# Madhudorai/encodec-pytorch

Hardware: AMD Instinct MI355X
Metric: audio-seconds/sec EnCodec24k train step, batch 32x1s (higher is better)
Workload: dtype f32; 1 GPU; config 3: 24 kHz mono full GAN (MS-STFT disc + Balancer); global_batch=32, parallelism=dp1

## Files before the change

### encodec-pytorch_amd/csrc/conv2d.h

```cpp
#pragma once
#include "common.h"

constexpr int NT = 256;
constexpr int DPER = 8;

struct C2Geo {
    int B, Ci, T2, Fi, Co, Fo, KT, KF, sf, dt, pt, pf;
};
static inline bool geo_ok(const C2Geo& g) {
    return g.B > 0 && g.Ci > 0 && g.T2 > 0 && g.Fi > 0 && g.Co > 0 && g.Fo > 0 && g.KT > 0 && g.KF > 0 &&
           g.sf > 0 && g.dt > 0 && g.pt >= 0 && g.pf >= 0 &&
           g.Fo == (g.Fi + 2 * g.pf - g.KF) / g.sf + 1 && g.T2 + 2 * g.pt - g.dt * (g.KT - 1) == g.T2;
}

static inline int c2_rows(int BN, int len) { return (len + BN - 2) / len + 1; }

static inline int c2_ck(int VC, int per_ch, int budget = 12288) {
    int ck = budget / per_ch;
    if (ck > 32) ck = 32;
    int vce = (VC + 1) & ~1;
    if (ck > vce) ck = vce;
    ck &= ~1;
    if (ck < 2) ck = 2;
    for (int c = ck; c >= 2; c -= 2)
        if (VC % c == 0 && c * 2 >= ck) return c;
    return ck;
}

static inline int quad_ck(int VC, int NR, int RL, int MQ, int CKM) {
    const int quads = NR * (((RL + 3) & ~3) >> 2);
    int ck = MQ * NT / quads;
    ck = std::min(ck, CKM);
    ck = std::min(ck, (VC + 1) & ~1);
    ck &= ~1;
    return ck;
}

extern int g_c2_select;
bool rw_pays(int64_t items, int64_t positions, double ratio);

ENCX_DEV f32x4 quad_abs(f32x4 v, int o, int last) {
    const int sh = o < 0 ? o : (o > last ? o - last : 0);
    const int n = sh < 0 ? -sh : sh;
    const bool b1 = n & 1, b2 = n & 2;
    f32x4 r;
    if (sh >= 0) {
        const float t0 = b1 ? v[1] : v[0], t1 = b1 ? v[2] : v[1], t2 = b1 ? v[3] : v[2], t3 = b1 ? 0.f : v[3];
        r[0] = b2 ? t2 : t0;
        r[1] = b2 ? t3 : t1;
        r[2] = b2 ? 0.f : t2;
        r[3] = b2 ? 0.f : t3;
    } else {
        const float t0 = b1 ? 0.f : v[0], t1 = b1 ? v[0] : v[1], t2 = b1 ? v[1] : v[2], t3 = b1 ? v[2] : v[3];
        r[0] = b2 ? 0.f : t0;
        r[1] = b2 ? 0.f : t1;
        r[2] = b2 ? t0 : t2;
        r[3] = b2 ? t1 : t3;
    }
    return r;
}

ENCX_DEV int rw_first_slot(int wave) { return wave * (int)gridDim.x + xcd_linear_id(); }
```

### encodec-pytorch_amd/csrc/conv2d_fwd.hip

```cpp
#include "common.h"
#include "conv2d.h"
#include "prof.h"

namespace {

struct C2Fwd {
    C2Geo g;
    const float* x;
    const float* wf;
    const float* bias;
    float* y;
    int act;
    int CK, NR, RL;
};

template <int BM, int BN, int WM, int WN, int KFC = 0>
__global__ __launch_bounds__(NT) void c2_fwd_kernel(C2Fwd a) {
    constexpr int TM = BM / WM / 32, TN = BN / WN / 32;
    extern __shared__ float smem[];
    const C2Geo g = a.g;
    const int CK = a.CK, NR = a.NR, RL = a.RL, KF = g.KF, S = g.sf;
    const int VC = g.Ci * g.KT, XR = NR * RL;
    float* Xs = smem;
    float* Ws = smem + CK * XR;
    const int tid = threadIdx.x, lane = tid & 63, wave = tid >> 6;
    const int wm0 = (wave / WN) * TM * 32, wn0 = (wave % WN) * TN * 32;
    const int h = lane >> 5, l32 = lane & 31;
    const int b = blockIdx.z, n0 = blockIdx.x * BN, co0 = blockIdx.y * BM;
    const int Nall = g.T2 * g.Fo, nend = min(Nall, n0 + BN);
    const int tf = n0 / g.Fo, f0 = n0 - tf * g.Fo;
    const int nr = (nend - 1) / g.Fo - tf + 1;
    int boff[TN];
#pragma unroll
    for (int j = 0; j < TN; ++j) {
        const int n = n0 + wn0 + j * 32 + l32;
        boff[j] = 0;
        if (n < nend) {
            const int tr = n / g.Fo, f = n - tr * g.Fo, rs = tr - tf;
            boff[j] = rs * RL + (f - (rs ? 0 : f0)) * S;
        }
    }
    f32x16 acc[TM][TN];
#pragma unroll
    for (int i = 0; i < TM; ++i)
#pragma unroll
        for (int j = 0; j < TN; ++j) acc[i][j] = (f32x16){0};
    const float* xb = a.x + (int64_t)b * g.Ci * g.T2 * g.Fi;
    int2* rtab = (int2*)(Ws + KF * CK * BM);
    for (int gr = tid; gr < VC * NR; gr += NT) {
        const int vc = gr / NR, rs = gr - vc * NR, ci = vc / g.KT, kt = vc - ci * g.KT;
        const int row = tf + rs + kt * g.dt - g.pt, pos0 = (rs ? 0 : f0) * S - g.pf;
        const bool ok = rs < nr && row >= 0 && row < g.T2;
        rtab[gr] = make_int2(ok ? (ci * g.T2 + row) * g.Fi + pos0 : 0, ok ? pos0 : -(1 << 30));
    }
    const int dr = NT / RL, dw = NT - dr * RL, r_init = tid / RL, w_init = tid - r_init * RL;
    const int wcol = tid & (BM - 1);
    for (int c0 = 0; c0 < VC; c0 += CK) {
        __syncthreads();
        {
            const int nrows = min(CK, VC - c0) * NR, items = CK * XR;
            int r = r_init, w = w_init;
            for (int i0 = 0; i0 < items; i0 += NT * DPER) {
                int rq[DPER], wq[DPER];
#pragma unroll
                for (int q = 0; q < DPER; ++q) {
                    rq[q] = r;
                    wq[q] = w;
                    w += dw;
                    r += dr;
                    if (w >= RL) {
                        w -= RL;
                        ++r;
                    }
                }
                int2 e[DPER];
#pragma unroll
                for (int q = 0; q < DPER; ++q) e[q] = rtab[c0 * NR + (rq[q] < nrows ? rq[q] : 0)];
                float v[DPER];
#pragma unroll
                for (int q = 0; q < DPER; ++q) {
                    const int pos = e[q].y + wq[q];
                    const bool ok = rq[q] < nrows && pos >= 0 && pos < g.Fi;
                    const float t = xb[ok ? e[q].x + wq[q] : 0];
                    v[q] = ok ? t : 0.f;
                }
#pragma unroll
                for (int q = 0; q < DPER; ++q) {
                    const int i = i0 + q * NT + tid;
                    if (i < items) Xs[i] = v[q];
                }
            }
        }
        {
            const int items = KF * CK * BM, rows = (VC - c0) * KF, co = co0 + wcol;
            const float* wsrc = a.wf + (int64_t)c0 * KF * g.Co + co;
            for (int i0 = 0; i0 < items; i0 += NT * DPER) {
                float v[DPER];
#pragma unroll
                for (int q = 0; q < DPER; ++q) {
                    const int rr = (i0 + q * NT + tid) / BM;
                    const bool ok = rr < rows && co < g.Co;
                    const float t = wsrc[ok ? (int64_t)rr * g.Co : 0];
                    v[q] = ok ? t : 0.f;
                }
#pragma unroll
                for (int q = 0; q < DPER; ++q) {
                    const int i = i0 + q * NT + tid;
                    if (i < items) Ws[i] = v[q];
                }
            }
        }
        __syncthreads();
        if constexpr (KFC > 0) {
            for (int cp = 0; cp < CK; cp += 2) {
                const float* wk = Ws + (cp + h) * KFC * BM + wm0 + l32;
                const float* xk = Xs + (cp + h) * XR;
#pragma unroll
                for (int kf = 0; kf < KFC; ++kf) {
                    float av[TM], bv[TN];
#pragma unroll
                    for (int i = 0; i < TM; ++i) av[i] = wk[kf * BM + i * 32];
#pragma unroll
                    for (int j = 0; j < TN; ++j) bv[j] = xk[boff[j] + kf];
#pragma unroll
                    for (int i = 0; i < TM; ++i)
#pragma unroll
                        for (int j = 0; j < TN; ++j) acc[i][j] = mfma32(av[i], bv[j], acc[i][j]);
                }
            }
        } else {
            for (int kf = 0; kf < KF; ++kf) {
                const float* wk = Ws + (h * KF + kf) * BM + wm0 + l32;
                const float* xk = Xs + h * XR + kf;
                for (int cp = 0; cp < CK; cp += 2) {
                    float av[TM], bv[TN];
#pragma unroll
                    for (int i = 0; i < TM; ++i) av[i] = wk[cp * KF * BM + i * 32];
#pragma unroll
                    for (int j = 0; j < TN; ++j) bv[j] = xk[cp * XR + boff[j]];
#pragma unroll
                    for (int i = 0; i < TM; ++i)
#pragma unroll
                        for (int j = 0; j < TN; ++j) acc[i][j] = mfma32(av[i], bv[j], acc[i][j]);
                }
            }
        }
    }
#pragma unroll
    for (int i = 0; i < TM; ++i)
#pragma unroll
        for (int j = 0; j < TN; ++j) {
            const int n = n0 + wn0 + j * 32 + l32;
#pragma unroll
            for (int r = 0; r < 16; ++r) {
                const int co = co0 + wm0 + i * 32 + mfma_row(r, lane);
                const float bco = a.bias ? a.bias[co < g.Co ? co : g.Co - 1] : 0.f;
                if (co < g.Co && n < nend) {
                    float v = acc[i][j][r] + bco;
                    if (a.act) v = lrelu(v);
                    a.y[((int64_t)b * g.Co + co) * Nall + n] = v;
                }
            }
        }
}

template <int BN, int KFC, int MQ, int CKM, int OCC = 1>
__global__ __launch_bounds__(NT, OCC) void c2_fwdr_kernel(C2Fwd a) {
    constexpr int BM = 32, TN = BN / 128, MW = (KFC * CKM * BM / 4 + NT - 1) / NT;
    extern __shared__ float smem[];
    const C2Geo g = a.g;
    const int CK = a.CK, NR = a.NR, RL = a.RL, S = g.sf;
    const int RLp = (RL + 3) & ~3, NQ = RLp >> 2;
    const int VC = g.Ci * g.KT, XR = NR * RLp, WQ = KFC * CK * BM / 4;
    float* Xs = smem;
    float* Ws = smem + CK * XR;
    int2* rtab = (int2*)(Ws + KFC * CK * BM);
    const int tid = threadIdx.x, lane = tid & 63, wave = tid >> 6;
    const int h = lane >> 5, l32 = lane & 31;
    const TileId tile = xcd_tile();
    const int b = tile.z, n0 = tile.x * BN, co0 = tile.y * BM;
    const int wn0 = wave * TN * 32;
    const int Nall = g.T2 * g.Fo, nend = min(Nall, n0 + BN);
    const int tf = n0 / g.Fo, f0 = n0 - tf * g.Fo;
    const int nr = (nend - 1) / g.Fo - tf + 1;
    const int base0 = ((f0 * S - g.pf) & ~3), baseN = ((-g.pf) & ~3);
    int boff[TN];
#pragma unroll
    for (int j = 0; j < TN; ++j) {
        const int n = n0 + wn0 + j * 32 + l32;
        boff[j] = 0;
        if (n < nend) {
            const int tr = n / g.Fo, f = n - tr * g.Fo, rs = tr - tf;
            boff[j] = rs * RLp + f * S - g.pf - (rs ? baseN : base0);
        }
    }
    f32x16 acc[TN];
#pragma unroll
    for (int j = 0; j < TN; ++j) acc[j] = (f32x16){0};
    const int64_t xtot = (int64_t)g.B * g.Ci * g.T2 * g.Fi;
    const float* xb = a.x + (int64_t)b * g.Ci * g.T2 * g.Fi;
    const int64_t xleft = xtot - (int64_t)b * g.Ci * g.T2 * g.Fi;
    for (int gr = tid; gr < VC * NR; gr += NT) {
        const int vc = gr / NR, rs = gr - vc * NR, ci = vc / g.KT, kt = vc - ci * g.KT;
        const int row = tf + rs + kt * g.dt - g.pt, base = rs ? baseN : base0;
        const bool ok = rs < nr && row >= 0 && row < g.T2;
        rtab[gr] = make_int2(ok ? (ci * g.T2 + row) * g.Fi + base : 0, ok ? base : -(1 << 30));
    }
    __syncthreads();
    const int rows = CK * NR;
    const int dr = NT / NQ, dq = NT - dr * NQ, r_init = tid / NQ, q_init = tid - r_init * NQ;
    f32x4 xv[MQ], wv[MW];
    int xmask[MQ], xdst[MQ];
    auto fetch = [&](int c0) {
        const int nrows = min(CK, VC - c0) * NR;
        int r = r_init, q = q_init;
#pragma unroll
        for (int u = 0; u < MQ; ++u) {
            const bool live = r < nrows;
            const int2 e = rtab[c0 * NR + (live ? r : 0)];
            const int col = e.y + 4 * q;
            const bool any = live && col >= 0 && col < g.Fi;
            int off = any ? e.x + 4 * q : 0;
            if (off > xleft - 4) off = (int)xleft - 4;
            xv[u] = ld4u(xb + off);
            const int sh = (any ? e.x + 4 * q : 0) - off;
            xmask[u] = any ? (min(g.Fi - col, 4) | (sh << 4)) : 0;
            xdst[u] = r < rows ? r * RLp + 4 * q : -1;
            q += dq;
            r += dr;
            if (q >= NQ) {
                q -= NQ;
                ++r;
            }
        }
        const float* wsrc = a.wf + (int64_t)c0 * KFC * g.Co + co0;
        const int wrows = (VC - c0) * KFC;
#pragma unroll
        for (int u = 0; u < MW; ++u) {
            const int j = u * NT + tid, rr = j >> 3, col = (j & 7) * 4;
            const bool ok = j < WQ && rr < wrows && co0 + col + 3 < g.Co;
            wv[u] = ld4u(wsrc + (ok ? (int64_t)rr * g.Co + col : 0));
            if (!ok) wv[u] = (f32x4){0.f, 0.f, 0.f, 0.f};
        }
    };
    fetch(0);
    for (int c0 = 0; c0 < VC; c0 += CK) {
        __syncthreads();
#pragma unroll
        for (int u = 0; u < MQ; ++u) {
            const int m = xmask[u], nv = m & 15, sh = m >> 4;
            f32x4 v = xv[u];
            if (sh) {
                const f32x4 t = v;
#pragma unroll
                for (int k = 0; k < 4; ++k) v[k] = k + sh < 4 ? (k + sh == 1 ? t[1] : k + sh == 2 ? t[2] : t[3]) : 0.f;
            }
#pragma unroll
            for (int k = 0; k < 4; ++k) v[k] = k < nv ? v[k] : 0.f;
            if (xdst[u] >= 0) *(f32x4*)(Xs + xdst[u]) = v;
        }
#pragma unroll
        for (int u = 0; u < MW; ++u) {
            const int j = u * NT + tid, rr = j >> 3, col = (j & 7) * 4;
            if (j < WQ && rr < (VC - c0) * KFC && co0 + col + 3 >= g.Co)
                for (int k = 0; k < 4; ++k)
                    wv[u][k] = co0 + col + k < g.Co ? a.wf[((int64_t)c0 * KFC + rr) * g.Co + co0 + col + k] : 0.f;
            if (j < WQ) *(f32x4*)(Ws + rr * BM + col) = wv[u];
        }
        __syncthreads();
        if (c0 + CK < VC) fetch(c0 + CK);
#pragma unroll 2
        for (int cp = 0; cp < CK; cp += 2) {
            const float* wk = Ws + (cp + h) * KFC * BM + l32;
            const float* xk = Xs + (cp + h) * XR;
#pragma unroll
            for (int kf = 0; kf < KFC; ++kf) {
                const float av = wk[kf * BM];
                float bv[TN];
#pragma unroll
                for (int j = 0; j < TN; ++j) bv[j] = xk[boff[j] + kf];
#pragma unroll
                for (int j = 0; j < TN; ++j) acc[j] = mfma32(av, bv[j], acc[j]);
            }
        }
    }
#pragma unroll
    for (int j = 0; j < TN; ++j) {
        const int n = n0 + wn0 + j * 32 + l32;
#pragma unroll
        for (int r = 0; r < 16; ++r) {
            const int co = co0 + mfma_row(r, lane);
            const float bco = a.bias ? a.bias[co < g.Co ? co : g.Co - 1] : 0.f;
            if (co < g.Co && n < nend) {
                float v = acc[j][r] + bco;
                if (a.act) v = lrelu(v);
                a.y[((int64_t)b * g.Co + co) * Nall + n] = v;
            }
        }
    }
}

struct C2FwdR {
    C2Geo g;
    const float* x;
    const float* wf;
    const float* bias;
    float* y;
    int act;
    int F4;
    int tiles;
};
template <int KF, int S, int WQ, int NWV>
__global__ __launch_bounds__(NWV * 64) void c2_fwd_rw_kernel(C2FwdR a) {
    constexpr int NE = 4 * WQ, KT = 3;
    extern __shared__ float smem[];
    const C2Geo g = a.g;
    float* Ws = smem;
    float* Bs = smem + g.Ci * KT * KF * 32;
    for (int i = threadIdx.x; i < g.Ci * KT * KF * 32; i += NWV * 64) {
        const int co = i & 31, r = i >> 5;
        Ws[i] = co < g.Co ? a.wf[r * g.Co + co] : 0.f;
    }
    if (threadIdx.x < 32) Bs[threadIdx.x] = (a.bias && (int)threadIdx.x < g.Co) ? a.bias[threadIdx.x] : 0.f;
    __syncthreads();
    const int lane = threadIdx.x & 63, wave = threadIdx.x >> 6, h = lane >> 5, l = lane & 31;
    const int quads = g.B * g.T2 * a.F4;
    const int plane = g.T2 * g.Fi, xlast = g.B * g.Ci * plane - 4;
    const int CP = g.Ci >> 1;
    const int cstride = 2 * plane;
    struct Geo {
        int t, b, f0;
        int rb[KT];
        uint32_t msk[KT];
        bool fix;
    };
    auto geo = [&](int tile) {
        Geo q;
        const int qd = min(tile * 32 + l, quads - 1);
        const int fq = qd % a.F4, bt = qd / a.F4;
        q.t = bt % g.T2;
        q.b = bt / g.T2;
        q.f0 = 4 * fq;
        const int col0 = S * q.f0 - g.pf;
        uint32_t cmask = 0;
#pragma unroll
        for (int e = 0; e < NE; ++e) cmask |= (col0 + e >= 0 && col0 + e < g.Fi) ? (1u << e) : 0u;
        bool clean = true;
#pragma unroll
        for (int kt = 0; kt < KT; ++kt) {
            const int row = q.t + kt * g.dt - g.pt;
            const bool ok = row >= 0 && row < g.T2;
            q.rb[kt] = (q.b * g.Ci + h) * plane + (ok ? row : 0) * g.Fi + col0;
            q.msk[kt] = ok ? cmask : 0u;
            clean = clean && q.msk[kt] == (1u << NE) - 1;
        }
        q.fix = !__all(clean);
        return q;
    };
    auto load = [&](f32x4* w, const Geo& q, int c, int kt) {
        const int base = q.rb[kt] + c * cstride;
#pragma unroll
        for (int w4 = 0; w4 < WQ; ++w4) w[w4] = ld4u(a.x + min(max(base + 4 * w4, 0), xlast));
    };
    f32x4 wb[KT][WQ];
    auto wcol = [&](int c, int kt) { return Ws + ((2 * c + h) * KT + kt) * KF * 32 + l; };
    const int stride = gridDim.x * NWV;
    int tile = rw_first_slot(wave);
    if (tile < a.tiles) load(wb[0], geo(tile), 0, 0);
    for (; tile < a.tiles; tile += stride) {
        const Geo cur = geo(tile);
        const int t = cur.t, b = cur.b, f0 = cur.f0;
        f32x16 acc[4];
#pragma unroll
        for (int j = 0; j < 4; ++j) acc[j] = (f32x16){0};
        for (int c = 0; c < CP; ++c) {
#pragma unroll
            for (int kt = 0; kt < KT; ++kt) {
                const int nk = kt + 1 < KT ? kt + 1 : 0;
                if (kt + 1 < KT) load(wb[nk], cur, c, nk);
                else if (c + 1 < CP) load(wb[0], cur, c + 1, 0);
                else load(wb[0], geo(tile + stride < a.tiles ? tile + stride : tile), 0, 0);
                f32x4* w = wb[kt];
                if (cur.fix) {
                    const int base = cur.rb[kt] + c * cstride;
#pragma unroll
                    for (int q = 0; q < WQ; ++q) {
                        const int o = base + 4 * q;
                        if (__any(o < 0 || o > xlast)) w[q] = quad_abs(w[q], o, xlast);
#pragma unroll
                        for (int e = 0; e < 4; ++e)
                            if (!((cur.msk[kt] >> (4 * q + e)) & 1u)) w[q][e] = 0.f;
                    }
                }
                const float* wk = wcol(c, kt);
#pragma unroll
                for (int kf = 0; kf < KF; ++kf) {
                    const float av = wk[kf * 32];
#pragma unroll
                    for (int j = 0; j < 4; ++j) {
                        const int r = S * j + kf;
                        acc[j] = mfma32(av, w[r >> 2][r & 3], acc[j]);
                    }
                }
            }
        }
        if (tile * 32 + l < quads) {
#pragma unroll
            for (int r = 0; r < 16; ++r) {
                const int co = mfma_row(r, lane);
                if (co >= g.Co) continue;
                const float bco = Bs[co];
                f32x4 v;
#pragma unroll
                for (int j = 0; j < 4; ++j) {
                    const float u = acc[j][r] + bco;
                    v[j] = a.act ? lrelu(u) : u;
                }
                float* dst = a.y + (((int64_t)b * g.Co + co) * g.T2 + t) * g.Fo + f0;
                if (f0 + 4 <= g.Fo) {
                    *(f32x4u*)dst = v;
                } else {
#pragma unroll
                    for (int j = 0; j < 4; ++j)
                        if (f0 + j < g.Fo) dst[j] = v[j];
                }
            }
        }
    }
}


template <int KT, int KF, int S>
__global__ __launch_bounds__(256) void c2_co1_fwd(C2Fwd a) {
    const C2Geo g = a.g;
    __shared__ float part[4][64];
    const int lane = threadIdx.x & 63, cg = threadIdx.x >> 6;
    const int plane = g.T2 * g.Fo, p = blockIdx.x * 64 + lane, b = blockIdx.y;
    const int pc = p < plane ? p : plane - 1;
    const int t = pc / g.Fo, fo = pc - t * g.Fo;
    const int64_t xplane = (int64_t)g.T2 * g.Fi;
    const int cper = (g.Ci + 3) >> 2, c0 = cg * cper, c1 = min(g.Ci, c0 + cper);
    const int fb = fo * S - g.pf;
    float acc = 0.f;
    for (int ci = c0; ci < c1; ++ci) {
        const float* xc = a.x + ((int64_t)b * g.Ci + ci) * xplane;
        const float* w = a.wf + ci * KT * KF;
#pragma unroll
        for (int kt = 0; kt < KT; ++kt) {
            const int tr = t + kt * g.dt - g.pt;
            const bool rok = tr >= 0 && tr < g.T2;
            const float* row = xc + (int64_t)(rok ? tr : 0) * g.Fi;
#pragma unroll
            for (int kf = 0; kf < KF; ++kf) {
                const int f = fb + kf;
                const bool ok = rok && f >= 0 && f < g.Fi;
                const float v = row[ok ? f : 0];
                acc = fmaf(w[kt * KF + kf], ok ? v : 0.f, acc);
            }
        }
    }
    part[cg][lane] = acc;
    __syncthreads();
    if (cg == 0 && p < plane) {
        float v = ((part[0][lane] + part[1][lane]) + part[2][lane]) + part[3][lane];
        if (a.bias) v += a.bias[0];
        a.y[(int64_t)b * plane + p] = a.act ? lrelu(v) : v;
    }
}

template <int BM, int BN, int WM, int WN, int KFC = 0>
int launch_fwd(C2Fwd a, hipStream_t st) {
    const size_t lds = ((size_t)a.CK * a.NR * a.RL + (size_t)a.g.KF * a.CK * BM +
                        (size_t)2 * a.g.Ci * a.g.KT * a.NR + 2) * sizeof(float);
    dim3 grid((unsigned)cdiv((int64_t)a.g.T2 * a.g.Fo, BN), (unsigned)cdiv(a.g.Co, BM), (unsigned)a.g.B);
    hipLaunchKernelGGL((c2_fwd_kernel<BM, BN, WM, WN, KFC>), grid, dim3(NT), lds, st, a);
    ENCX_CHECK_LAUNCH();
    return 0;
}

template <int BM, int BN, int WM, int WN, int KFC = 0>
int run_fwd(C2Fwd a, hipStream_t st, int budget = 12288) {
    a.NR = c2_rows(BN, a.g.Fo);
    a.RL = (min(BN, a.g.Fo) - 1) * a.g.sf + a.g.KF;
    a.CK = c2_ck(a.g.Ci * a.g.KT, a.NR * a.RL + a.g.KF * BM, budget);
    return launch_fwd<BM, BN, WM, WN, KFC>(a, st);
}

static bool fwr_ok(const C2Geo& g) {
    if (g.Co > 32 || (g.Ci & 1) || g.KT != 3 || g.Fo < 1 || g.Fi < 4) return false;
    if ((int64_t)g.B * g.Ci * g.T2 * g.Fi >= (1ll << 31) || (int64_t)g.B * g.T2 * cdiv(g.Fo, 4) >= (1ll << 31) - 64)
        return false;
    if (!((g.KF == 9 && (g.sf == 2 || g.sf == 1)) || (g.KF == 3 && g.sf == 1))) return false;
    return (size_t)g.Ci * g.KT * g.KF * 32 * sizeof(float) <= 128 * 1024;
}
static int run_fwd_rw(const C2Fwd& f, int wgs, hipStream_t st) {
    if (!fwr_ok(f.g)) return ENCX_EINVAL;
    constexpr int NWV = 8;
    const C2Geo& g = f.g;
    C2FwdR a{g, f.x, f.wf, f.bias, f.y, f.act, (int)cdiv(g.Fo, 4), 0};
    a.tiles = (int)cdiv((int64_t)g.B * g.T2 * a.F4, 32);
    const size_t lds = ((size_t)g.Ci * g.KT * g.KF * 32 + 32) * sizeof(float);
    const int grid = (int)min((int64_t)wgs, cdiv(a.tiles, NWV));
    if (g.KF == 9 && g.sf == 2)
        hipLaunchKernelGGL((c2_fwd_rw_kernel<9, 2, 4, NWV>), dim3(grid), dim3(NWV * 64), lds, st, a);
    else if (g.KF == 9)
        hipLaunchKernelGGL((c2_fwd_rw_kernel<9, 1, 3, NWV>), dim3(grid), dim3(NWV * 64), lds, st, a);
    else
        hipLaunchKernelGGL((c2_fwd_rw_kernel<3, 1, 2, NWV>), dim3(grid), dim3(NWV * 64), lds, st, a);
    ENCX_CHECK_LAUNCH();
    return 0;
}
template <int BN, int KFC, int MQ, int CKM, int OCC = 1>
int run_fwdr(C2Fwd a, hipStream_t st) {
    a.NR = c2_rows(BN, a.g.Fo);
    a.RL = (min(BN, a.g.Fo) - 1) * a.g.sf + a.g.KF + 3;
    a.CK = quad_ck(a.g.Ci * a.g.KT, a.NR, a.RL, MQ, CKM);
    if (a.g.KF != KFC || a.CK < 2 || a.g.Fi < 4 || a.g.pf > 4) return ENCX_EINVAL;
    const int RLp = (a.RL + 3) & ~3;
    const size_t lds = ((size_t)a.CK * a.NR * RLp + (size_t)KFC * a.CK * 32 + (size_t)2 * a.g.Ci * a.g.KT * a.NR) *
                       sizeof(float);
    dim3 grid((unsigned)cdiv((int64_t)a.g.T2 * a.g.Fo, BN), (unsigned)cdiv(a.g.Co, 32), (unsigned)a.g.B);
    hipLaunchKernelGGL((c2_fwdr_kernel<BN, KFC, MQ, CKM, OCC>), grid, dim3(NT), lds, st, a);
    ENCX_CHECK_LAUNCH();
    return 0;
}

}

int g_c2_select = [] {
    const char* v = getenv("ENCX_C2");
    return v ? atoi(v) : 0;
}();
bool rw_pays(int64_t items, int64_t positions, double ratio) {
    if (g_c2_select != 0) return g_c2_select == 1;
    static const int simds = [] {
        int cus = 0;
        if (hipDeviceGetAttribute(&cus, hipDeviceAttributeMultiprocessorCount, 0) != hipSuccess || cus <= 0) cus = 256;
        return 4 * cus;
    }();
    const double rounds = std::ceil((double)items / simds), tiled = (double)positions / (128.0 * simds);
    return rounds < ratio * tiled;
}

extern "C" {

int encx_conv2d_select(int mode) {
    const int prev = g_c2_select;
    if (mode >= 0 && mode <= 2) g_c2_select = mode;
    return prev;
}

int encx_conv2d_fwd(const float* x, const float* wf, const float* bias, float* y, int64_t B, int64_t Ci,
                    int64_t T2, int64_t Fi, int64_t Co, int64_t Fo, int64_t KT, int64_t KF, int64_t sf,
                    int64_t dt, int64_t pt, int64_t pf, int act, encx_stream_t stream) {
    ENCX_REQUIRE(x && wf && y);
    C2Geo g{(int)B, (int)Ci, (int)T2, (int)Fi, (int)Co, (int)Fo, (int)KT, (int)KF, (int)sf, (int)dt, (int)pt, (int)pf};
    ENCX_REQUIRE(geo_ok(g));
    hipStream_t st = (hipStream_t)stream;
    encx_prof_scope ps(st, 2.0 * B * Co * T2 * Fo * Ci * KT * KF, 4.0 * (B * Ci * T2 * Fi + B * Co * T2 * Fo), "c2_fwd");
    ps.tag(" %ldx%ld %ldx%ld s%ld T%ld F%ld", (long)Ci, (long)Co, (long)KT, (long)KF, (long)sf, (long)T2, (long)Fo);
    C2Fwd a{g, x, wf, bias, y, act, 0, 0, 0};
    const int fw_wgs = (int)encx_opt(OPT_FWR);
    if (fw_wgs > 0 && fwr_ok(g) &&
        ((Ci * KT < 16 && g_c2_select != 2) || rw_pays(cdiv(B * T2 * cdiv(Fo, 4), 32), B * T2 * Fo, 87.0 / 66.0)) &&
        run_fwd_rw(a, fw_wgs, st) == 0)
        return 0;
    if (Co == 1 && KT == 3 && KF == 3 && (sf == 1 || sf == 2)) {
        dim3 grid((unsigned)cdiv(T2 * Fo, 64), (unsigned)B);
        if (sf == 1) hipLaunchKernelGGL((c2_co1_fwd<3, 3, 1>), grid, dim3(256), 0, st, a);
        else hipLaunchKernelGGL((c2_co1_fwd<3, 3, 2>), grid, dim3(256), 0, st, a);
        ENCX_CHECK_LAUNCH();
        return 0;
    }
    if (Co <= 32 && Ci * KT >= 16) {
        if (KF == 9 && run_fwdr<256, 9, 6, 16>(a, st) == 0) return 0;
        if (KF == 3 && run_fwdr<256, 3, 6, 32>(a, st) == 0) return 0;
    }
    if (Co <= 32) return run_fwd<32, 128, 1, 4>(a, st);
    return run_fwd<64, 128, 2, 2>(a, st);
}

}
```

### encodec-pytorch_amd/csrc/conv2d_wgrad.hip

```cpp
#include "common.h"
#include "conv2d.h"
#include "prof.h"

namespace {

constexpr int WG_BT = 64;

struct C2Wg {
    C2Geo g;
    const float* dy;
    const float* yact;
    const float* x;
    float* ws;
    int BT, NR, RL, NCmax, items, per_split, chunks;
};

template <int BM, int BN, int WM, int WN, int WK, bool YM = true>
__global__ __launch_bounds__(NT) void c2_wgrad_kernel(C2Wg a) {
    constexpr int TM = BM / WM / 32, TN = BN / WN / 32;
    static_assert(WM * WN * WK == 4, "4 waves");
    extern __shared__ float smem[];
    const C2Geo g = a.g;
    constexpr int BT = WG_BT;
    const int NR = a.NR, RL = a.RL, KF = g.KF, S = g.sf;
// ... 54 lines not shown
                if (YM) ym[q] = ysrc[o];
                v[q] = ok ? t : 0.f;
            }
#pragma unroll
            for (int q = 0; q < DPER; ++q) {
                const int i = i0 + q * NT + tid;
                if (i < BT * BM) {
                    const int tl = i % BT, col = i / BT;
                    Ls[tl * BM + col] = YM ? v[q] * lrelu_grad(ym[q]) : v[q];
                }
            }
        }
        {
            const int items = a.NCmax * XR, nrows = a.NCmax * NR, tfo = tf * g.Fi;
            int r = r_init, w = w_init;
            for (int i0 = 0; i0 < items; i0 += NT * DPER) {
                int rq[DPER], wq[DPER];
#pragma unroll
                for (int q = 0; q < DPER; ++q) {
                    rq[q] = r;
                    wq[q] = w;
                    w += dw;
                    r += dr;
                    if (w >= RL) {
                        w -= RL;
                        ++r;
                    }
                }
                int4 e[DPER];
#pragma unroll
                for (int q = 0; q < DPER; ++q) e[q] = rtab[rq[q] < nrows ? rq[q] : 0];
                float v[DPER];
#pragma unroll
                for (int q = 0; q < DPER; ++q) {
                    const int row = tf + e[q].y, pos = (e[q].z ? 0 : f0) * S - g.pf + wq[q];
                    const bool ok = rq[q] < nrows && e[q].w && e[q].z < nr && row >= 0 && row < g.T2 && pos >= 0 &&
                                    pos < g.Fi;
                    const float t = xb[ok ? e[q].x + tfo + pos : 0];
                    v[q] = ok ? t : 0.f;
                }
#pragma unroll
                for (int q = 0; q < DPER; ++q) {
                    const int i = i0 + q * NT + tid;
                    if (i < items) Rs[i] = v[q];
                }
            }
        }
        for (int tl = tid; tl < BT; tl += NT) {
            const int p = p0 + tl;
            int off = 0;
            if (p < pend) {
                const int tr = p / g.Fo, f = p - tr * g.Fo, rs = tr - tf;
                off = rs * RL + (f - (rs ? 0 : f0)) * S;
            }
            poff[tl] = off;
        }
        __syncthreads();
        for (int tp = wk * tw; tp < (wk + 1) * tw; tp += 2) {
            const int tl = tp + h;
            const int po = poff[tl];
            float av[TM], bv[TN];
#pragma unroll
            for (int i = 0; i < TM; ++i) av[i] = Ls[tl * BM + wm0 + i * 32 + l32];
#pragma unroll
            for (int j = 0; j < TN; ++j) bv[j] = isb[j] ? 1.f : Rs[cbase[j] + po];
#pragma unroll
            for (int i = 0; i < TM; ++i)
#pragma unroll
                for (int j = 0; j < TN; ++j) acc[i][j] = mfma32(av[i], bv[j], acc[i][j]);
        }
    }
    if (WK > 1) {
        __syncthreads();
        float* red = smem;
#pragma unroll
        for (int i = 0; i < TM; ++i)
#pragma unroll
            for (int j = 0; j < TN; ++j)
#pragma unroll
                for (int r = 0; r < 16; ++r)
                    red[(((wmn * WK + wk) * TM * TN + i * TN + j) * 16 + r) * 64 + lane] = acc[i][j][r];
        __syncthreads();
        if (wk != 0) return;
#pragma unroll
        for (int i = 0; i < TM; ++i)
#pragma unroll
            for (int j = 0; j < TN; ++j)
#pragma unroll
                for (int r = 0; r < 16; ++r) {
                    float v = red[(((wmn * WK) * TM * TN + i * TN + j) * 16 + r) * 64 + lane];
                    for (int w = 1; w < WK; ++w)
                        v += red[(((wmn * WK + w) * TM * TN + i * TN + j) * 16 + r) * 64 + lane];
                    acc[i][j][r] = v;
                }
    }
    float* wsb = a.ws + (int64_t)split * g.Co * N;
#pragma unroll
    for (int i = 0; i < TM; ++i)
#pragma unroll
        for (int j = 0; j < TN; ++j) {
            const int n = n0 + wn0 + j * 32 + l32;
#pragma unroll
            for (int r = 0; r < 16; ++r) {
                const int co = co0 + wm0 + i * 32 + mfma_row(r, lane);
                if (co < g.Co && n < N) wsb[(int64_t)co * N + n] = acc[i][j][r];
            }
        }
}

constexpr int W3_P = 64;
struct C2Wg3 {
    C2Geo g;
    const float* dy;
    const float* yact;
    const float* x;
    float* ws;
    int NR, RL, GC, items, per_split, chunks;
};
template <int KF, int NTW, int NW, int MQ, int ML, int OCC = 1, bool YM = true>
__global__ __launch_bounds__(NW * 64, OCC) void c2_wgrad3_kernel(C2Wg3 a) {
    constexpr int NTH = NW * 64, P = W3_P, LDA = 33, PQ = P / 4;
    extern __shared__ float smem[];
    const C2Geo g = a.g;
    const int NR = a.NR, RL = a.RL, GC = a.GC, S = g.sf;
    const int RLp = (RL + 3) & ~3, NQ = RLp >> 2, XR = NR * RLp;
    const int VC = g.Ci * g.KT, Nw = VC * KF, N = Nw + 1;
    int4* rtab = (int4*)smem;
    float* Ls = smem + 4 * GC * NR;
    int* poff = (int*)(Ls + P * LDA);
    float* Rs = (float*)(poff + P);
    const int tid = threadIdx.x, lane = tid & 63, wave = tid >> 6;
    const int h = lane >> 5, l32 = lane & 31;
    const TileId tile = xcd_tile();
    const int vc0 = tile.x * GC, split = tile.y;
    const int n0 = vc0 * KF + wave * NTW * 32;
    const int Nall = g.T2 * g.Fo;
    const int64_t plane_y = (int64_t)Nall, plane_x = (int64_t)g.T2 * g.Fi;
    const int64_t ytot = (int64_t)g.B * g.Co * plane_y, xtot = (int64_t)g.B * g.Ci * plane_x;
    const bool do_bias = tile.x == 0 && wave == 0;
    const int baseN = (-g.pf) & ~3;
    int cbase[NTW];
#pragma unroll
    for (int j = 0; j < NTW; ++j) {
        const int n = n0 + j * 32 + l32;
        const int vc = n / KF, kf = n - vc * KF;
        cbase[j] = (n < Nw) ? (vc - vc0) * XR + kf : 0;
    }
    f32x16 acc[NTW];
#pragma unroll
    for (int j = 0; j < NTW; ++j) acc[j] = (f32x16){0};
    float bsum = 0.f;
    for (int r = tid; r < GC * NR; r += NTH) {
        const int cl = r / NR, rs = r - cl * NR, vc = vc0 + cl, ci = vc / g.KT, kt = vc - ci * g.KT;
        const int rrel = rs + kt * g.dt - g.pt;
        rtab[r] = make_int4(ci * (int)plane_x + rrel * g.Fi, rrel, rs, vc < VC);
    }
    const int dr = NTH / NQ, dq = NTH - dr * NQ, r_init = tid / NQ, q_init = tid - r_init * NQ;
    const int it_beg = split * a.per_split, it_end = min(a.items, it_beg + a.per_split);
    __syncthreads();
    f32x4 dv[ML], yv[ML], xv[MQ];
    int dmask[ML], xmask[MQ];
    auto load = [&](int it) {
        const int b = it / a.chunks, p0 = (it - b * a.chunks) * P;
        const int pend = min(Nall, p0 + P);
        const int tf = p0 / g.Fo, f0 = p0 - tf * g.Fo;
        const int nr = (pend - 1) / g.Fo - tf + 1;
        const int base0 = (f0 * S - g.pf) & ~3;
        const int64_t yb = (int64_t)b * g.Co * plane_y, xbo = (int64_t)b * g.Ci * plane_x;
#pragma unroll
        for (int u = 0; u < ML; ++u) {
            const int i = u * NTH + tid, co = i / PQ, k = i - co * PQ, p = p0 + 4 * k;
            const bool any = i < 32 * PQ && co < g.Co && p < pend;
            int64_t off = any ? yb + (int64_t)co * plane_y + p : 0;
            const int64_t offc = off > ytot - 4 ? ytot - 4 : off;
            dv[u] = ld4u(a.dy + offc);
            if (YM) yv[u] = ld4u(a.yact + offc);
            dmask[u] = any ? (min(pend - p, 4) | ((int)(off - offc) << 4)) : 0;
        }
        int r = r_init, q = q_init;
#pragma unroll
        for (int u = 0; u < MQ; ++u) {
            const int rr = r < GC * NR ? r : 0;
            const int4 e = rtab[rr];
            const int base = e.z ? baseN : base0, col = base + 4 * q;
            const int row = tf + e.y;
            const bool any = r < GC * NR && e.w && e.z < nr && row >= 0 && row < g.T2 && col >= 0 && col < g.Fi;
            int64_t off = any ? xbo + e.x + (int64_t)tf * g.Fi + col : 0;
            const int64_t offc = off > xtot - 4 ? xtot - 4 : off;
            xv[u] = ld4u(a.x + offc);
            xmask[u] = any ? (min(g.Fi - col, 4) | ((int)(off - offc) << 4)) : 0;
            q += dq;
            r += dr;
            if (q >= NQ) {
                q -= NQ;
                ++r;
            }
        }
    };
    auto store = [&](int it) {
        const int b = it / a.chunks, p0 = (it - b * a.chunks) * P;
        const int pend = min(Nall, p0 + P);
        const int tf = p0 / g.Fo, f0 = p0 - tf * g.Fo;
        const int base0 = (f0 * S - g.pf) & ~3;
#pragma unroll
        for (int u = 0; u < ML; ++u) {
            const int i = u * NTH + tid, co = i / PQ, k = i - co * PQ;
            if (i < 32 * PQ) {
                const int m = dmask[u], nv = m & 15, sh = m >> 4;
                f32x4 v = dv[u], y = yv[u];
                if (sh) {
                    const f32x4 t = v, ty = y;
#pragma unroll
                    for (int c = 0; c < 4; ++c) {
                        v[c] = c + sh < 4 ? (c + sh == 1 ? t[1] : c + sh == 2 ? t[2] : t[3]) : 0.f;
                        y[c] = c + sh < 4 ? (c + sh == 1 ? ty[1] : c + sh == 2 ? ty[2] : ty[3]) : 0.f;
                    }
                }
#pragma unroll
                for (int c = 0; c < 4; ++c)
                    Ls[(4 * k + c) * LDA + co] = c < nv ? (YM ? v[c] * lrelu_grad(y[c]) : v[c]) : 0.f;
            }
        }
        int r = r_init, q = q_init;
#pragma unroll
        for (int u = 0; u < MQ; ++u) {
            const int m = xmask[u], nv = m & 15, sh = m >> 4;
            f32x4 v = xv[u];
            if (sh) {
                const f32x4 t = v;
#pragma unroll
                for (int c = 0; c < 4; ++c) v[c] = c + sh < 4 ? (c + sh == 1 ? t[1] : c + sh == 2 ? t[2] : t[3]) : 0.f;
            }
#pragma unroll
            for (int c = 0; c < 4; ++c) v[c] = c < nv ? v[c] : 0.f;
            if (r < GC * NR) *(f32x4*)(Rs + r * RLp + 4 * q) = v;
            q += dq;
            r += dr;
            if (q >= NQ) {
                q -= NQ;
                ++r;
            }
        }
        for (int tl = tid; tl < P; tl += NTH) {
            const int p = p0 + tl;
            int off = 0;
            if (p < pend) {
                const int tr = p / g.Fo, f = p - tr * g.Fo, rs = tr - tf;
                off = rs * RLp + f * S - g.pf - (rs ? baseN : base0);
            }
            poff[tl] = off;
        }
    };
    for (int it = it_beg; it < it_end; ++it) {
        load(it);
        __syncthreads();
        store(it);
        __syncthreads();
#pragma unroll 4
        for (int kp = 0; kp < P / 2; ++kp) {
            const int tl = 2 * kp + h;
            const int po = poff[tl];
            const float av = Ls[tl * LDA + l32];
            bsum += av;
            float bv[NTW];
#pragma unroll
            for (int j = 0; j < NTW; ++j) bv[j] = Rs[cbase[j] + po];
#pragma unroll
            for (int j = 0; j < NTW; ++j) acc[j] = mfma32(av, bv[j], acc[j]);
        }
    }
    float* wsb = a.ws + (int64_t)split * g.Co * N;
#pragma unroll
    for (int j = 0; j < NTW; ++j) {
        const int n = n0 + j * 32 + l32;
#pragma unroll
        for (int r = 0; r < 16; ++r) {
            const int co = mfma_row(r, lane);
            if (co < g.Co && n < Nw) wsb[(int64_t)co * N + n] = acc[j][r];
        }
    }
    if (do_bias) {
        bsum += __shfl_xor(bsum, 32, 64);
        if (h == 0 && l32 < g.Co) wsb[(int64_t)l32 * N + Nw] = bsum;
    }
}

struct C2WgR {
    C2Geo g;
    const float* dy;
    const float* yact;
    const float* x;
    float* ws;
    int NC;
    int items;
    int per_split;
    int ktg;
    int cib;
    int SW, NCS;
};
template <int KTW, int WQ>
struct RwStage {
    f32x4 av, yv, xw[KTW][WQ];
};
ENCX_DEV f32x4 ld4_sv(const float* base, uint32_t lane_bytes, int imm = 0) {
    typedef const __attribute__((address_space(1))) char* gptr;
    const uint64_t b = (uint64_t)base;
    const uint32_t lo = __builtin_amdgcn_readfirstlane((uint32_t)b);
    const uint32_t hi = __builtin_amdgcn_readfirstlane((uint32_t)(b >> 32));
    const gptr p = (gptr)(((uint64_t)hi << 32) | lo);
    return *(const __attribute__((address_space(1))) f32x4u*)(p + (uint64_t)lane_bytes + imm);
}
struct RwPos {
    int cs, t, strip, b;
};
template <int KTW>
struct RwItem {
    int f0;
    int sy;
    int sx[KTW];
    bool edge;
    bool rok[KTW];
    bool ends;
};
template <int KF, int S, int KTW, int WQ, bool YM, int NW = 1>
__global__ __launch_bounds__(NW * 64, NW == 1 ? 2 : 1) void c2_wgrad_rw_kernel(C2WgR a) {
    constexpr int NTAP = KTW * KF;
    static_assert(NW == 1 || NW == 8, "one-wave or 8-wave workgroups");
    const C2Geo g = a.g;
    const int lane = threadIdx.x & 63, h = lane >> 5, l = lane & 31;
    const int wv = __builtin_amdgcn_readfirstlane((int)(threadIdx.x >> 6));
    const int id = xcd_linear_id();
    const int kg = id % a.ktg, rest = id / a.ktg, cb = rest % a.cib, split = rest / a.cib;
    const int kt0 = kg * KTW, ci = cb * 32 + l;
    const bool ci_ok = ci < g.Ci, co_ok = l < g.Co;
    const bool full = g.Co >= 32 && (cb + 1) * 32 <= g.Ci;
    const int it_beg = split * a.per_split, it_end = min(a.items, it_beg + a.per_split);
    const int plane_y = g.T2 * g.Fo, plane_x = g.T2 * g.Fi;
    const int ylast = g.B * g.Co * plane_y - 4, xlast = g.B * g.Ci * plane_x - 4;
    f32x16 acc[NTAP];
#pragma unroll
    for (int j = 0; j < NTAP; ++j) acc[j] = (f32x16){0};
    float bsum = 0.f;
    auto advance = [&](RwPos& q) {
        q.cs += NW;
        while (q.cs >= a.SW) {
            q.cs -= a.SW;
            if (++q.t == g.T2) {
                q.t = 0;
                if (++q.strip == a.NCS) {
                    q.strip = 0;
                    ++q.b;
                }
            }
        }
    };
    const int ly = (co_ok ? l : 0) * plane_y + 4 * h;
    const int lx = (ci_ok ? ci : 0) * plane_x + 4 * S * h;
    const int ly_max = (min(g.Co, 32) - 1) * plane_y + 4;
    const int lx_max = min(g.Ci - 1, cb * 32 + 31) * plane_x + 4 * S;
    const bool sv_ok = g.Co * plane_y < (1 << 29) && g.Ci * plane_x < (1 << 29) && plane_y >= 8 &&
                       plane_x >= 4 * S + 4 * WQ;
    const uint32_t lyb = sv_ok ? 4u * (uint32_t)ly : 0u, lxb = sv_ok ? 4u * (uint32_t)lx : 0u;
    auto item = [&](const RwPos& q) {
        RwItem<KTW> it;
        const int f0 = (q.strip * a.SW + q.cs) * 8;
        it.f0 = f0;
        it.sy = q.b * g.Co * plane_y + q.t * g.Fo + f0;
        const int xb = q.b * g.Ci * plane_x + S * f0 - g.pf;
#pragma unroll
        for (int k = 0; k < KTW; ++k) {
            const int row = q.t + (kt0 + k) * g.dt - g.pt;
            it.rok[k] = row >= 0 && row < g.T2;
            it.sx[k] = xb + (it.rok[k] ? row : 0) * g.Fi;
        }
        it.edge = f0 + 8 > g.Fo || S * f0 - g.pf < 0 || S * (f0 + 4) - g.pf + 4 * WQ > g.Fi;
        it.ends = !sv_ok || it.sy + ly_max > ylast;
#pragma unroll
        for (int k = 0; k < KTW; ++k) it.ends = it.ends || it.sx[k] < 0 || it.sx[k] + lx_max + 4 * (WQ - 1) > xlast;
        return it;
    };
    auto load_in = [&](RwStage<KTW, WQ>& st, const RwItem<KTW>& it) {
        const int sy = it.ends ? 0 : it.sy;
        st.av = ld4_sv(a.dy + sy, lyb);
        if (YM) st.yv = ld4_sv(a.yact + sy, lyb);
#pragma unroll
        for (int k = 0; k < KTW; ++k) {
            const int sx = it.ends ? 0 : it.sx[k];
#pragma unroll
            for (int w = 0; w < WQ; ++w) st.xw[k][w] = ld4_sv(a.x + sx, lxb, 16 * w);
        }
    };
    auto load_any = [&](RwStage<KTW, WQ>& st, const RwItem<KTW>& it) {
        const int oac = min(it.sy + ly, ylast);
        st.av = ld4u(a.dy + oac);
        if (YM) st.yv = ld4u(a.yact + oac);
#pragma unroll
        for (int k = 0; k < KTW; ++k) {
            const int rb = it.sx[k] + lx;
#pragma unroll
            for (int w = 0; w < WQ; ++w) st.xw[k][w] = ld4u(a.x + min(max(rb + 4 * w, 0), xlast));
        }
    };
    auto fix = [&](RwStage<KTW, WQ>& st, const RwItem<KTW>& it) {
        if (it.edge) {
            const int p = it.f0 + 4 * h, col0 = S * p - g.pf;
            const int oa = it.sy + ly;
            if (__any(oa > ylast)) {
                st.av = quad_abs(st.av, oa, ylast);
                if (YM) st.yv = quad_abs(st.yv, oa, ylast);
            }
#pragma unroll
            for (int e = 0; e < 4; ++e)
                if (p + e >= g.Fo) st.av[e] = 0.f;
#pragma unroll
            for (int w = 0; w < WQ; ++w) {
#pragma unroll
                for (int k = 0; k < KTW; ++k) {
                    const int o = it.sx[k] + lx + 4 * w;
                    if (__any(o < 0 || o > xlast)) st.xw[k][w] = quad_abs(st.xw[k][w], o, xlast);
                }
#pragma unroll
                for (int e = 0; e < 4; ++e) {
                    const int col = col0 + 4 * w + e;
                    if (col < 0 || col >= g.Fi) {
#pragma unroll
                        for (int k = 0; k < KTW; ++k) st.xw[k][w][e] = 0.f;
                    }
                }
            }
        }
        if (!full) {
            if (!co_ok) st.av = (f32x4){0.f, 0.f, 0.f, 0.f};
#pragma unroll
            for (int k = 0; k < KTW; ++k)
#pragma unroll
                for (int w = 0; w < WQ; ++w)
                    if (!ci_ok) st.xw[k][w] = (f32x4){0.f, 0.f, 0.f, 0.f};
        }
    };
    auto grad = [&](const RwStage<KTW, WQ>& st) {
#pragma clang fp contract(off)
        f32x4 ca = st.av;
        if (YM) {
#pragma unroll
            for (int e = 0; e < 4; ++e) ca[e] *= lrelu_grad(st.yv[e]);
        }
        bsum += (ca[0] + ca[1]) + (ca[2] + ca[3]);
        return ca;
    };
    auto taps = [&](const RwStage<KTW, WQ>& st, const f32x4& ca, int k) {
#pragma unroll
        for (int q = 0; q < 4; ++q)
#pragma unroll
            for (int kf = 0; kf < KF; ++kf) {
                const int r = S * q + kf;
                acc[k * KF + kf] = mfma32(ca[q], st.xw[k][r >> 2][r & 3], acc[k * KF + kf]);
            }
    };
    auto step = [&](RwStage<KTW, WQ>& sc, const RwItem<KTW>& cu, RwStage<KTW, WQ>& sn, const RwItem<KTW>& nx) {
        if (cu.edge || !full) fix(sc, cu);
        constexpr int KM = KTW / 2;
        f32x4 ca;
        if (cu.rok[KM]) {
            load_in(sn, nx);
            __builtin_amdgcn_fence(__ATOMIC_RELEASE, "wavefront");
            __builtin_amdgcn_sched_barrier(0);
            ca = grad(sc);
            taps(sc, ca, KM);
        } else {
            load_in(sn, nx);
            __builtin_amdgcn_fence(__ATOMIC_RELEASE, "wavefront");
            __builtin_amdgcn_sched_barrier(0);
            ca = grad(sc);
        }
#pragma unroll
        for (int k = 0; k < KTW; ++k)
            if (k != KM && cu.rok[k]) taps(sc, ca, k);
        if (nx.ends) load_any(sn, nx);
    };
    RwStage<KTW, WQ> s0, s1;
    const int it0 = it_beg + wv;
    if (it0 < it_end) {
        RwPos pos;
        const int r1 = it0 / a.SW, r2 = r1 / g.T2;
        pos.cs = it0 - r1 * a.SW;
        pos.t = r1 - r2 * g.T2;
        pos.b = r2 / a.NCS;
        pos.strip = r2 - pos.b * a.NCS;
        RwItem<KTW> i0 = item(pos), i1;
        load_any(s0, i0);
        for (int it = it0;; it += 2 * NW) {
            if (it + NW < it_end) advance(pos);
            i1 = item(pos);
            step(s0, i0, s1, i1);
            if (it + NW >= it_end) break;
            if (it + 2 * NW < it_end) advance(pos);
            i0 = item(pos);
            step(s1, i1, s0, i0);
            if (it + 2 * NW >= it_end) break;
        }
    }
    if constexpr (NW > 1) {
        extern __shared__ float red[];
        constexpr int TS = 32 * 32 * NTAP;
        float* bred = red + 4 * TS;
        bsum += __shfl_xor(bsum, 32, 64);
        if (h == 0) bred[wv * 32 + l] = bsum;
#pragma unroll
        for (int pass = 0; pass < 2; ++pass) {
            if ((wv >> 2) == pass) {
                float* reg = red + (wv & 3) * TS;
#pragma unroll
                for (int r = 0; r < 16; ++r) {
                    const int co = mfma_row(r, lane);
#pragma unroll
                    for (int j = 0; j < NTAP; ++j) {
                        float* q = reg + (co * 32 + l) * NTAP + j;
                        *q = pass == 0 ? acc[j][r] : *q + acc[j][r];
                    }
                }
            }
            __syncthreads();
        }
        const int64_t SZ = (int64_t)a.ktg * a.cib * TS + 32;
        float* dst = a.ws + (int64_t)split * SZ + (int64_t)(kg * a.cib + cb) * TS;
        for (int d = threadIdx.x; d < TS; d += NW * 64)
            dst[d] = ((red[d] + red[TS + d]) + red[2 * TS + d]) + red[3 * TS + d];
        if (kg == 0 && cb == 0 && threadIdx.x < 32) {
            float b = 0.f;
#pragma unroll
            for (int w = 0; w < NW; ++w) b += bred[w * 32 + threadIdx.x];
            a.ws[(int64_t)split * SZ + (SZ - 32) + threadIdx.x] = b;
        }
        return;
    }
    const int N = g.Ci * g.KT * KF + 1;
    float* wsb = a.ws + (int64_t)split * g.Co * N;
    if (ci_ok) {
#pragma unroll
        for (int r = 0; r < 16; ++r) {
            const int co = mfma_row(r, lane);
            if (co < g.Co) {
                float* dst = wsb + (int64_t)co * N + (ci * g.KT + kt0) * KF;
#pragma unroll
                for (int j = 0; j < NTAP; ++j) dst[j] = acc[j][r];
            }
        }
    }
    if (kg == 0 && cb == 0) {
        bsum += __shfl_xor(bsum, 32, 64);
        if (h == 0 && co_ok) wsb[(int64_t)l * N + N - 1] = bsum;
    }
}

__global__ __launch_bounds__(256) void c2_slab_group_sum(const float* ws, int S, int G, int64_t n, float* part) {
    const int64_t i = (int64_t)blockIdx.x * 256 + threadIdx.x;
    if (i >= n) return;
    const int g = blockIdx.y, s0 = g * G, cnt = min(G, S - s0);
    part[(int64_t)g * n + i] = (float)sum_strided_d(ws + (int64_t)s0 * n + i, cnt, n);
}

__global__ __launch_bounds__(256) void c2_wg_reduce(const float* ws, int S, int Co, int N, float* dw, float* db,
                                                    int acc_w, int acc_b) {
    __shared__ double red[256];
    const int64_t i = (int64_t)blockIdx.x * 64 + (threadIdx.x & 63);
    const bool valid = i < (int64_t)Co * N;
    const float v = slab_sum_256_d(ws + (valid ? i : 0), S, (int64_t)Co * N, valid, red);
    if (threadIdx.x >= 64 || !valid) return;
    const int co = (int)(i / N), n = (int)(i - (int64_t)co * N);
    const int Nw = N - 1;
    if (n < Nw) {
        if (dw) {
            float* p = dw + (int64_t)co * Nw + n;
            *p = acc_w ? *p + v : v;
        }
    } else if (db) {
        db[co] = acc_b ? db[co] + v : v;
    }
}

__global__ __launch_bounds__(256) void c2_wgr_reduce(const float* ws, int S, int64_t SZ, int Co, int Ci, int KT,
                                                     int KF, int KTW, int cib, float* dw, float* db, int acc_w,
                                                     int acc_b) {
    __shared__ double red[256];
    const int N = Ci * KT * KF + 1;
    const int64_t i = (int64_t)blockIdx.x * 64 + (threadIdx.x & 63);
    const bool valid = i < (int64_t)Co * N;
    int64_t off = 0;
    int co = 0, n = 0;
    if (valid) {
        co = (int)(i / N);
        n = (int)(i - (int64_t)co * N);
        if (n < N - 1) {
            const int ci = n / (KT * KF), kt = (n / KF) % KT, kf = n % KF;
            const int kg = kt / KTW, k = kt % KTW, NTAP = KTW * KF;
            off = ((((int64_t)kg * cib + ci / 32) * 32 + co) * 32 + (ci & 31)) * NTAP + k * KF + kf;
        } else {
            off = SZ - 32 + co;
        }
    }
    const float v = slab_sum_256_d(ws + off, S, SZ, valid, red);
    if (threadIdx.x >= 64 || !valid) return;
    if (n < N - 1) {
        if (dw) {
            float* p = dw + (int64_t)co * (N - 1) + n;
            *p = acc_w ? *p + v : v;
        }
    } else if (db) {
        db[co] = acc_b ? db[co] + v : v;
    }
}

template <int KT, int KF, int S>
__global__ __launch_bounds__(256) void c2_co1_wgrad(C2Wg a) {
// ... 311 lines not shown
```

Baseline: 957.4 audio-seconds/sec.

## Deepen load prefetch and use scalar-base loads in register-window conv2d forward

Reworks the register-window conv2d forward kernel so input loads are issued two steps ahead by default instead of one, and weight values for the next step are loaded from shared memory during the current MFMA loop. Interior tiles use scalar-base plus lane-offset global loads with no clamping, and masking is done branch-free with bit operations. Clamping and shifting stay only for tiles that touch tensor ends. The aim is to hide memory latency and cut address arithmetic in the MFMA loop, at the cost of more registers and scheduling barriers that could reduce occupancy.

Result: no change. 959.5 audio-seconds/sec, median of 6 (+0.2%).

```diff
diff --git a/encodec-pytorch_amd/csrc/conv2d.h b/encodec-pytorch_amd/csrc/conv2d.h
--- a/encodec-pytorch_amd/csrc/conv2d.h
+++ b/encodec-pytorch_amd/csrc/conv2d.h
@@ -60,4 +60,22 @@
     return r;
 }
 
+ENCX_DEV f32x4 ld4_sv(const float* base, uint32_t lane_bytes, int imm = 0) {
+    typedef const __attribute__((address_space(1))) char* gptr;
+    const uint64_t b = (uint64_t)base;
+    const uint32_t lo = __builtin_amdgcn_readfirstlane((uint32_t)b);
+    const uint32_t hi = __builtin_amdgcn_readfirstlane((uint32_t)(b >> 32));
+    const gptr p = (gptr)(((uint64_t)hi << 32) | lo);
+    return *(const __attribute__((address_space(1))) f32x4u*)(p + (uint64_t)lane_bytes + imm);
+}
+
+ENCX_DEV float keep_bit(float v, uint32_t msk, int i) {
+    return __int_as_float(__float_as_int(v) & ((int)(msk << (31 - i)) >> 31));
+}
+
+ENCX_DEV void pin_loads() {
+    __builtin_amdgcn_fence(__ATOMIC_RELEASE, "wavefront");
+    __builtin_amdgcn_sched_barrier(0);
+}
+
 ENCX_DEV int rw_first_slot(int wave) { return wave * (int)gridDim.x + xcd_linear_id(); }
diff --git a/encodec-pytorch_amd/csrc/conv2d_fwd.hip b/encodec-pytorch_amd/csrc/conv2d_fwd.hip
--- a/encodec-pytorch_amd/csrc/conv2d_fwd.hip
+++ b/encodec-pytorch_amd/csrc/conv2d_fwd.hip
@@ -300,6 +300,9 @@
     }
 }
 
+#ifndef ENCX_FWR_PF
+#define ENCX_FWR_PF 2
+#endif
 struct C2FwdR {
     C2Geo g;
     const float* x;
@@ -328,11 +331,16 @@
     const int plane = g.T2 * g.Fi, xlast = g.B * g.Ci * plane - 4;
     const int CP = g.Ci >> 1;
     const int cstride = 2 * plane;
+    const bool sv_ok = (int64_t)g.B * g.Ci * plane < (1ll << 30);
     struct Geo {
         int t, b, f0;
-        int rb[KT];
+        uint32_t lo[KT];
         uint32_t msk[KT];
-        bool fix;
+        bool ends;
+    };
+    auto rbase = [&](int t, int b, int f0, int kt) {
+        const int row = t + kt * g.dt - g.pt;
+        return (b * g.Ci + h) * plane + (row >= 0 && row < g.T2 ? row : 0) * g.Fi + S * f0 - g.pf;
     };
     auto geo = [&](int tile) {
         Geo q;
@@ -345,30 +353,44 @@
         uint32_t cmask = 0;
 #pragma unroll
         for (int e = 0; e < NE; ++e) cmask |= (col0 + e >= 0 && col0 + e < g.Fi) ? (1u << e) : 0u;
-        bool clean = true;
+        bool out = false;
 #pragma unroll
         for (int kt = 0; kt < KT; ++kt) {
             const int row = q.t + kt * g.dt - g.pt;
-            const bool ok = row >= 0 && row < g.T2;
-            q.rb[kt] = (q.b * g.Ci + h) * plane + (ok ? row : 0) * g.Fi + col0;
-            q.msk[kt] = ok ? cmask : 0u;
-            clean = clean && q.msk[kt] == (1u << NE) - 1;
-        }
-        q.fix = !__all(clean);
+            const int rb = rbase(q.t, q.b, q.f0, kt);
+            q.msk[kt] = (row >= 0 && row < g.T2) ? cmask : 0u;
+            q.lo[kt] = 4u * (uint32_t)rb;
+            out = out || rb < 0 || rb + (CP - 1) * cstride + 4 * (WQ - 1) > xlast;
+        }
+        q.ends = !sv_ok || __any(out);
         return q;
     };
-    auto load = [&](f32x4* w, const Geo& q, int c, int kt) {
-        const int base = q.rb[kt] + c * cstride;
-#pragma unroll
-        for (int w4 = 0; w4 < WQ; ++w4) w[w4] = ld4u(a.x + min(max(base + 4 * w4, 0), xlast));
+    auto load = [&](f32x4* w, uint32_t lo, int c, bool ends, int t, int b, int f0, int kt) {
+        if (ends) {
+            const int rb = rbase(t, b, f0, kt) + c * cstride;
+#pragma unroll
+            for (int w4 = 0; w4 < WQ; ++w4) w[w4] = ld4u(a.x + min(max(rb + 4 * w4, 0), xlast));
+        } else {
+            const float* base = a.x + c * cstride;
+#pragma unroll
+            for (int w4 = 0; w4 < WQ; ++w4) w[w4] = ld4_sv(base, lo, 16 * w4);
+        }
     };
+    constexpr int PF = ENCX_FWR_PF;
+    static_assert(PF == 1 || PF == 2, "prefetch distance in steps");
     f32x4 wb[KT][WQ];
+    float av[KF];
     auto wcol = [&](int c, int kt) { return Ws + ((2 * c + h) * KT + kt) * KF * 32 + l; };
     const int stride = gridDim.x * NWV;
     int tile = rw_first_slot(wave);
-    if (tile < a.tiles) load(wb[0], geo(tile), 0, 0);
+    if (tile >= a.tiles) return;
+    Geo cur = geo(tile);
+#pragma unroll
+    for (int kt = 0; kt < PF; ++kt) load(wb[kt], cur.lo[kt], 0, cur.ends, cur.t, cur.b, cur.f0, kt);
+#pragma unroll
+    for (int kf = 0; kf < KF; ++kf) av[kf] = wcol(0, 0)[kf * 32];
     for (; tile < a.tiles; tile += stride) {
-        const Geo cur = geo(tile);
+        const Geo nxt = geo(tile + stride < a.tiles ? tile + stride : tile);
         const int t = cur.t, b = cur.b, f0 = cur.f0;
         f32x16 acc[4];
 #pragma unroll
@@ -376,31 +398,33 @@
         for (int c = 0; c < CP; ++c) {
 #pragma unroll
             for (int kt = 0; kt < KT; ++kt) {
-                const int nk = kt + 1 < KT ? kt + 1 : 0;
-                if (kt + 1 < KT) load(wb[nk], cur, c, nk);
-                else if (c + 1 < CP) load(wb[0], cur, c + 1, 0);
-                else load(wb[0], geo(tile + stride < a.tiles ? tile + stride : tile), 0, 0);
+                const bool lastc = c + 1 == CP;
+                const int nk = (kt + PF) % KT;
+                const bool wrap = kt + PF >= KT, last = wrap && lastc;
+                const int cn = !wrap ? c : (last ? 0 : c + 1);
+                load(wb[nk], last ? nxt.lo[nk] : cur.lo[nk], cn, last ? nxt.ends : cur.ends, last ? nxt.t : cur.t,
+                     last ? nxt.b : cur.b, last ? nxt.f0 : cur.f0, nk);
+                pin_loads();
                 f32x4* w = wb[kt];
-                if (cur.fix) {
-                    const int base = cur.rb[kt] + c * cstride;
-#pragma unroll
-                    for (int q = 0; q < WQ; ++q) {
-                        const int o = base + 4 * q;
-                        if (__any(o < 0 || o > xlast)) w[q] = quad_abs(w[q], o, xlast);
-#pragma unroll
-                        for (int e = 0; e < 4; ++e)
-                            if (!((cur.msk[kt] >> (4 * q + e)) & 1u)) w[q][e] = 0.f;
-                    }
-                }
-                const float* wk = wcol(c, kt);
+                if (cur.ends) {
+                    const int rb = rbase(cur.t, cur.b, cur.f0, kt) + c * cstride;
+#pragma unroll
+                    for (int q = 0; q < WQ; ++q) w[q] = quad_abs(w[q], rb + 4 * q, xlast);
+                }
+#pragma unroll
+                for (int q = 0; q < WQ; ++q)
+#pragma unroll
+                    for (int e = 0; e < 4; ++e) w[q][e] = keep_bit(w[q][e], cur.msk[kt], 4 * q + e);
+                const float* wn = wcol(kt + 1 < KT ? c : (lastc ? 0 : c + 1), (kt + 1) % KT);
 #pragma unroll
                 for (int kf = 0; kf < KF; ++kf) {
-                    const float av = wk[kf * 32];
 #pragma unroll
                     for (int j = 0; j < 4; ++j) {
                         const int r = S * j + kf;
-                        acc[j] = mfma32(av, w[r >> 2][r & 3], acc[j]);
+                        acc[j] = mfma32(av[kf], w[r >> 2][r & 3], acc[j]);
                     }
+                    av[kf] = wn[kf * 32];
+                    __builtin_amdgcn_sched_barrier(0);
                 }
             }
         }
@@ -426,6 +450,7 @@
                 }
             }
         }
+        cur = nxt;
     }
 }
 
diff --git a/encodec-pytorch_amd/csrc/conv2d_wgrad.hip b/encodec-pytorch_amd/csrc/conv2d_wgrad.hip
--- a/encodec-pytorch_amd/csrc/conv2d_wgrad.hip
+++ b/encodec-pytorch_amd/csrc/conv2d_wgrad.hip
@@ -380,14 +380,6 @@
 struct RwStage {
     f32x4 av, yv, xw[KTW][WQ];
 };
-ENCX_DEV f32x4 ld4_sv(const float* base, uint32_t lane_bytes, int imm = 0) {
-    typedef const __attribute__((address_space(1))) char* gptr;
-    const uint64_t b = (uint64_t)base;
-    const uint32_t lo = __builtin_amdgcn_readfirstlane((uint32_t)b);
-    const uint32_t hi = __builtin_amdgcn_readfirstlane((uint32_t)(b >> 32));
-    const gptr p = (gptr)(((uint64_t)hi << 32) | lo);
-    return *(const __attribute__((address_space(1))) f32x4u*)(p + (uint64_t)lane_bytes + imm);
-}
 struct RwPos {
     int cs, t, strip, b;
 };
```
